# AechPro/Prism

Hardware: NVIDIA B200
Metric: PER sampled transitions/s (4 new steps ingested -> sample -> 3-step gather -> DQN update -> priority write-back, per learner iteration) (higher is better)
Workload: dtype f32

## Files before the change

### include/prism_b200.h

```cpp
#ifndef PRISM_B200_H
#define PRISM_B200_H

#include <stdint.h>

#ifdef __cplusplus
extern "C" {
#endif

#define PB_ABI_VERSION 2

enum {
    PB_OK = 0,
    PB_E_ARG = -1,
    PB_E_CAPACITY = -2,
    PB_E_UNSUPPORTED = -3,
    PB_E_POOL = -4
};

enum {
    PB_ST_EMPTY = 1,
    PB_ST_PSUM_NONPOS = 2,
    PB_ST_PMIN_NONPOS = 4
};

// ... 171 lines not shown
                         const unsigned long long *epoch, long long stride, float *partial_scratch,
                         long long *step_count, int *n_partials_out_h, void *stream);
int pb_pack_grads(int n_tensors, const long long *table, float scale, float *flat,
                  float *partial_scratch, long long *step_count, int *n_partials_out_h,
                  void *stream);
int pb_grad_sumsq(long long n, const float *grad, float *partial_scratch, long long *step_count,
                  int *n_partials_out_h, void *stream);
int pb_adam_clip_apply(long long n, float *param, const float *grad, float *exp_avg,
                       float *exp_avg_sq, const long long *step_count, float lr, float beta1,
                       float beta2, float adam_eps, float max_grad_norm,
                       const float *partial_scratch, int n_partials, float *norm_out,
                       void *stream);
long long pb_adam_fused_max_n(void);
int pb_adam_fused_step(int n_tensors, const long long *table, float scale, long long n, float *param, float *grad,
                       float *exp_avg, float *exp_avg_sq, long long *step_count, float lr, float beta1, float beta2,
                       float adam_eps, float max_grad_norm, float *partial_scratch, float *norm_out, void *stream);
int pb_adam_clip_step(long long n, float *param, const float *grad, float *exp_avg, float *exp_avg_sq,
                      long long *step_count, float lr, float beta1, float beta2, float adam_eps,
                      float max_grad_norm, float *norm_out, float *partial_scratch, void *stream);

int pb_conv3x3_relu_fwd(int B, int H, int W, int C, int OC, const float *x, const float *w,
                        const float *bias, float *out, void *stream);
int pb_conv3x3_relu_bwd_groups(int B);
int pb_conv3x3_relu_bwd(int B, int H, int W, int C, int OC, const float *x, const float *out,
                        const float *dout, float *partial_scratch, float *dw, float *db,
                        void *stream);

int pb_linear_fwd(int K, int M, int N, int J, const float *X, long long x_head_stride, const float *W,
                  const float *b, int act, float *Y, void *stream);
int pb_linear_bwd_input(int K, int M, int N, int J, const float *dY, const float *Ymask, const float *W,
                        int sum_heads, float *dX, void *stream);
int pb_linear_bwd_weight(int K, int M, int N, int J, const float *dY, const float *Ymask, const float *X,
                         long long x_head_stride, float *dW, float *db, void *stream);
int pb_gemm_trace(int enable, unsigned long long *out, int n_out);

int pb_tc_gemm_supported(int M, int N, int K, long long lda, long long ldb, long long ldc);
int pb_tc_gemm(int batch, int kbatches, int M, int N, int K,
               const float *A, int a_major, long long lda, long long a_bs,
               const float *B, int b_major, long long ldb, long long b_bs,
               const float *bias, long long bias_bs, int act,
               const float *mul, int mul_rows, long long ld_mul,
               float *C, long long ldc, long long c_bs,
               float *workspace, long long workspace_floats, int split_mode, void *stream);
int pb_linear_fwd_tc_supported(int M, int N, int J);
int pb_linear_fwd_tc(int K, int M, int N, int J, const float *X, long long x_head_stride, const float *W,
                     const float *b, int act, float *Y, void *stream);

int pb_iqn_phi_bwd(int n, int B, int F, const float *dh, const float *phi, const float *x, float *dpre, float *dx,
                   float *dbias_partial, void *stream);

#define PB_PEER_MAX 8
typedef struct pb_peer_group {
    int world, rank;
    float *grad[PB_PEER_MAX];
    float *reduced[PB_PEER_MAX];
    unsigned long long *flags[PB_PEER_MAX];
    double *norm_parts[PB_PEER_MAX];
    unsigned char *state[PB_PEER_MAX];
    unsigned long long *epoch;
    unsigned int *status;
    unsigned long long timeout_ns;
    long long grad_stride;
} pb_peer_group;
int pb_peer_alloc(long long bytes, void **ptr);
int pb_peer_free(void *ptr);
int pb_optimizer_preload(void);
// ... 75 lines not shown
```

### prism_b200/_lib.py

```python
import ctypes as C
import os

from . import build as _build

_LIB = None


class PbError(RuntimeError):
    pass


class pb_per_state(C.Structure):
    _fields_ = [
        ("len", C.c_longlong), ("seq", C.c_longlong), ("max_priority", C.c_float), ("p_sum", C.c_float),
        ("p_min", C.c_float), ("status", C.c_int), ("batch_max", C.c_float), ("owned_lo", C.c_int),
        ("owned_n", C.c_int), ("pad", C.c_int * 5),
    ]


class pb_tree(C.Structure):
    _fields_ = [
        ("sum", C.c_void_p), ("min", C.c_void_p), ("owner", C.c_void_p), ("counters", C.c_void_p),
        ("state", C.c_void_p),
        ("capacity", C.c_longlong), ("size", C.c_longlong), ("alpha", C.c_float), ("eps_f32", C.c_float),
# ... 102 lines not shown
    "pb_peer_pull_sum": [_PEER, _LL, _P, _P, C.POINTER(C.c_int), _P],
    "pb_peer_adam": [_PEER, _LL, _P, _P, _P, _P, _F, _F, _F, _F, _F, _P, _P, _P],
    "pb_peer_allreduce_adam_max_n": [],
    "pb_peer_two_phase_min": [_I],
    "pb_peer_allreduce_adam": [_PEER, _LL, _P, _P, _P, _P, _F, _F, _F, _F, _F, _P, _P, _P],
    "pb_peer_state_put": [_PEER, _P, _P],
    "pb_peer_trace": [_I, _P, _I],
    "pb_tree_sample_global_peer": [_TREE, _PEER, _LL, _P, _F, _P, _P, _P, _P],
    "pb_layer_norm_supported": [_LL, _I],
    "pb_layer_norm_bwd_blocks": [_LL, _I],
    "pb_layer_norm_fwd": [_LL, _I, _F, _P, _P, _P, _P, _P, _P, _P],
    "pb_layer_norm_bwd": [_LL, _I, _P, _P, _P, _P, _P, _P, _P, _P, _P, _P],
    "pb_layer_norm_grouped_fwd": [_I, _LL, _LL, _I, _F, _P, _P, _P, _P, _P, _P, _P],
    "pb_layer_norm_grouped_bwd_blocks": [_I, _LL, _I],
    "pb_layer_norm_grouped_bwd": [_I, _LL, _LL, _I, _P, _P, _P, _P, _P, _P, _P, _P, _P, _P],
    "pb_narrow_linear_supported": [_LL, _I, _I],
    "pb_narrow_linear_bwd_blocks": [_LL],
    "pb_narrow_linear_fwd": [_I, _LL, _I, _I, _P, _LL, _P, _P, _P, _P],
    "pb_narrow_linear_bwd": [_I, _LL, _I, _I, _P, _LL, _P, _P, _P, _P, _P, _P, _P],
    "pb_narrow_linear_bwd_reduce": [_I, _LL, _I, _I, _P, _P, _P, _P],
    "pb_sum_heads": [_I, _LL, _P, _P, _P],
    "pb_iqn_draw_cos_basis": [_LL, _I, _P, _P, _P, _P],
    "pb_relu_bwd_bias_strips": [_LL],
    "pb_relu_bwd_bias": [_I, _LL, _I, _P, _P, _P, _P, _P, _P],
    "pb_theil_chunks": [_LL],
    "pb_theil_fwd": [_I, _I, _I, _P, _P, _P, _P, _P],
    "pb_theil_bwd": [_I, _I, _I, _P, _P, _P, _P, _P],
    "pb_iqn_phi_bwd": [_I, _I, _I, _P, _P, _P, _P, _P, _P, _P],
    "pb_tc_gemm_supported": [_I, _I, _I, _LL, _LL, _LL],
    "pb_tc_gemm": [_I, _I, _I, _I, _I, _P, _I, _LL, _LL, _P, _I, _LL, _LL, _P, _LL, _I, _P, _I, _LL, _P, _LL, _LL, _P, _LL, _I, _P],
    "pb_linear_fwd_tc_supported": [_I, _I, _I],
    "pb_linear_fwd_tc": [_I, _I, _I, _I, _P, _LL, _P, _P, _I, _P, _P],
    "pb_linear_bwd_input": [_I, _I, _I, _I, _P, _P, _P, _I, _P, _P],
    "pb_linear_bwd_weight": [_I, _I, _I, _I, _P, _P, _P, _LL, _P, _P, _P],
    "pb_stamp_time": [_P, _P],
    "pb_store_stage_block": [_LL, _LL, _I, _LL, _LL, _LL, _P, _P, _P, _P, _I, _P, _P, _P, _P, _P, _P, _P, _P],
    "pb_wire_unpack_numbers": [_P, _LL, _P, _LL, _P],
    "pb_wire_array_header": [_LL, _P, _P],
    "pb_wire_pack_numbers": [_P, _I, _LL, _P, _LL, _P],
    "pb_wire_index_timesteps": [_P, _LL, _LL, _P, _P],
}
_RESTYPES = {"pb_error_string": C.c_char_p, "pb_launch_count": C.c_longlong, "pb_peer_slice": C.c_longlong,
             "pb_peer_allreduce_adam_max_n": C.c_longlong, "pb_adam_fused_max_n": C.c_longlong}

PB_E_POOL = -4
ABI_VERSION = 2


def lib_path():
    return _build.LIB_PATH


def load():
    global _LIB
    if _LIB is not None:
        return _LIB
    path = _build.build()
    if not os.path.exists(path):
        raise PbError("libprism_b200.so missing at %s and could not be built" % path)
    lib = C.CDLL(path)
    for name, argtypes in SIGNATURES.items():
        fn = getattr(lib, name)
        fn.argtypes = argtypes
        fn.restype = _RESTYPES.get(name, C.c_int)
    if lib.pb_abi_version() != ABI_VERSION:
        raise PbError("libprism_b200.so ABI version mismatch")
    _LIB = lib
    return lib


def check(rc, what=""):
    if rc != 0:
        msg = load().pb_error_string(rc).decode()
        raise PbError("%s failed: %s (code %d)" % (what or "libprism_b200 call", msg, rc))


def ptr(t):
# ... 16 lines not shown
```

### prism_b200/agents/ops.py

```python
import collections

import torch

from .. import _lib

ROUTES = collections.Counter()


def route_counts(reset=False):
    out = dict(ROUTES)
    if reset:
        ROUTES.clear()
    return out


def fallthrough_count():
    return sum(v for k, v in ROUTES.items() if k.startswith("fallthrough"))


def _c(t, dtype=torch.float32):
    if t.dtype != dtype:
        t = t.to(dtype)
    return t if t.is_contiguous() else t.contiguous()

# ... 141 lines not shown


def loss_combine(dist_loss, q_loss, per_weights):
    return _LossCombine.apply(dist_loss, q_loss, per_weights)


PARALLEL_BACKWARD = __import__('os').environ.get('PB_PARALLEL_BACKWARD', '1') != '0'
TRACE_MARK = None


def trace_mark(name):
    if TRACE_MARK is not None:
        TRACE_MARK(name)
_SIDE_STREAMS = {}


SERIAL_GRAPH = __import__('os').environ.get('PB_SERIAL_GRAPH', '0') == '1'


def fork_stream(device, key="bwd"):
    device = torch.device(device)
    if SERIAL_GRAPH:
        return torch.cuda.current_stream(device)
    s = _SIDE_STREAMS.get((device, key))
    if s is None:
        s = _SIDE_STREAMS[(device, key)] = torch.cuda.Stream(device=device)
    return s


def _side_stream(device):
    return fork_stream(device, "bwd")


_JOINS = {"mode": 0, "streams": [], "ptrs": []}


def defer_joins(mode):
    _JOINS["mode"], _JOINS["streams"], _JOINS["ptrs"] = int(mode), [], []


def finish_deferred(device):
    cur = torch.cuda.current_stream(device)
    seen = set()
    for s in _JOINS["streams"]:
        if s.cuda_stream not in seen and s.cuda_stream != cur.cuda_stream:
            seen.add(s.cuda_stream)
            cur.wait_stream(s)
    ptrs = _JOINS["ptrs"]
    defer_joins(0)
    return ptrs


def _join_or_defer(side, device, *grads):
    mode = _JOINS["mode"]
    if mode:
        _JOINS["ptrs"].extend(g.data_ptr() for g in grads if g is not None)
    if mode == 2:
        _JOINS["streams"].append(side)
    else:
        torch.cuda.current_stream(device).wait_stream(side)


class _Linear(torch.autograd.Function):

    @staticmethod
    def forward(ctx, x, w, b, act):
        _lib.require_cuda(x, "x")
        K, N, J = w.shape
        shared = x.dim() == 2
        M = x.shape[-2]
        xc, wc, bc = _c(x), _c(w), (None if b is None else _c(b))
        y = torch.empty(K, M, N, dtype=torch.float32, device=x.device)
        _lib.check(_lib.load().pb_linear_fwd(K, M, N, J, xc.data_ptr(), 0 if shared else M * J, wc.data_ptr(),
                                             _lib.ptr(bc), int(act), y.data_ptr(), _stream(x)), "pb_linear_fwd")
        ctx.act, ctx.shared, ctx.dims, ctx.has_bias = int(act), shared, (K, M, N, J), b is not None
        ctx.save_for_backward(xc, wc, y if act else None)
        return y

    @staticmethod
    def backward(ctx, dy):
        xc, wc, y = ctx.saved_tensors
        K, M, N, J = ctx.dims
        dy = _c(dy)
        lib, stream = _lib.load(), _stream(dy)
        mask = _lib.ptr(y) if ctx.act else None
        dx = dw = db = None
        want_dx = ctx.needs_input_grad[0]
        want_dw = ctx.needs_input_grad[1] or (ctx.has_bias and ctx.needs_input_grad[2])
        if want_dx:
            dx = torch.empty((M, J) if ctx.shared else (K, M, J), dtype=torch.float32, device=dy.device)
        if want_dw:
            dw = torch.empty(K, N, J, dtype=torch.float32, device=dy.device)
            db = torch.empty(K, N, dtype=torch.float32, device=dy.device) if ctx.has_bias else None
        side = _side_stream(dy.device) if (want_dx and want_dw and PARALLEL_BACKWARD) else None
        if want_dw:
            if side is not None:
                cur = torch.cuda.current_stream(dy.device)
                side.wait_stream(cur)
                with torch.cuda.stream(side):
                    _lib.check(lib.pb_linear_bwd_weight(K, M, N, J, dy.data_ptr(), mask, xc.data_ptr(),
                                                        0 if ctx.shared else M * J, dw.data_ptr(), _lib.ptr(db),
                                                        side.cuda_stream), "pb_linear_bwd_weight")
            else:
                _lib.check(lib.pb_linear_bwd_weight(K, M, N, J, dy.data_ptr(), mask, xc.data_ptr(),
                                                    0 if ctx.shared else M * J, dw.data_ptr(), _lib.ptr(db), stream),
                           "pb_linear_bwd_weight")
        if want_dx:
            _lib.check(lib.pb_linear_bwd_input(K, M, N, J, dy.data_ptr(), mask, wc.data_ptr(), int(ctx.shared),
                                               dx.data_ptr(), stream), "pb_linear_bwd_input")
        if side is not None:
            _join_or_defer(side, dy.device, dw, db)
        if TRACE_MARK is not None:
            TRACE_MARK("bwd:linear K%d M%d N%d J%d" % (K, M, N, J))
        return dx, dw, db, None


FUSED_LINEAR_MAX_ROWS = 512
NARROW_OUT, NARROW_MAX_ROWS = 32, 4096


_TC_WORKSPACE = {}
TC_WORKSPACE_FLOATS = 15 * 1024 * 1024
TC_SPLIT_MODE = 0


def _tc_workspace(device, stream):
    key = (device, stream)
    ws = _TC_WORKSPACE.get(key)
    if ws is None:
        ws = _TC_WORKSPACE[key] = torch.empty(TC_WORKSPACE_FLOATS, dtype=torch.float32, device=device)
    return ws


def tc_gemm(out, a, a_major, lda, a_bs, b, b_major, ldb, b_bs, batch, M, N, K, bias=None, bias_bs=0, act=0,
            kbatches=1, ldc=None, c_bs=None, mul=None):
    _lib.require_cuda(out, "out")
    stream = _stream(out)
    ws = _tc_workspace(out.device, stream)
    _lib.check(_lib.load().pb_tc_gemm(int(batch), int(kbatches), int(M), int(N), int(K),
                                      a.data_ptr(), int(a_major), int(lda), int(a_bs),
# ... 23 lines not shown
    @staticmethod
    def backward(ctx, dy):
        xc, wc, y = ctx.saved_tensors
        K, M, N, J = ctx.dims
        dy = _c(dy)
        lib = _lib.load()
        want_db = ctx.has_bias and ctx.needs_input_grad[2]
        dz, db = dy, None
        if ctx.act or want_db:
            strips = lib.pb_relu_bwd_bias_strips(M)
            partials = torch.empty(K * strips * N, dtype=torch.float32, device=dy.device)
            dz = torch.empty_like(dy) if ctx.act else dy
            db = torch.empty(K, N, dtype=torch.float32, device=dy.device) if want_db else None
            _lib.check(lib.pb_relu_bwd_bias(K, M, N, dy.data_ptr(), _lib.ptr(y) if ctx.act else None,
                                            dz.data_ptr() if ctx.act else None, _lib.ptr(db), partials.data_ptr(),
                                            _stream(dy)), "pb_relu_bwd_bias")
        dx = dw = None
        if ctx.needs_input_grad[0]:
            if ctx.shared:
                dx = torch.empty(M, J, dtype=torch.float32, device=dz.device)
                tc_gemm(dx, dz, 0, N, M * N, wc, 1, J, N * J, 1, M, J, N, kbatches=K)
            else:
                dx = torch.empty(K, M, J, dtype=torch.float32, device=dz.device)
                tc_gemm(dx, dz, 0, N, M * N, wc, 1, J, N * J, K, M, J, N)
        if ctx.needs_input_grad[1]:
            dw = torch.empty(K, N, J, dtype=torch.float32, device=dz.device)
            tc_gemm(dw, dz, 1, N, M * N, xc, 1, J, 0 if ctx.shared else M * J, K, N, J, M)
        return dx, dw, db, None


class _NarrowLinear(torch.autograd.Function):

    @staticmethod
    def forward(ctx, x, w, b):
        K, N, J = w.shape
        shared = x.dim() == 2
        M = x.shape[-2]
        xc, wc, bc = _c(x), _c(w), (None if b is None else _c(b))
        y = torch.empty(K, M, N, dtype=torch.float32, device=x.device)
        _lib.check(_lib.load().pb_narrow_linear_fwd(K, M, N, J, xc.data_ptr(), 0 if shared else M * J, wc.data_ptr(),
                                                    _lib.ptr(bc), y.data_ptr(), _stream(x)), "pb_narrow_linear_fwd")
        ctx.save_for_backward(xc, wc)
        ctx.has_bias, ctx.shared = b is not None, shared
        return y

    @staticmethod
    def backward(ctx, dy):
        xc, wc = ctx.saved_tensors
        K, N, J = wc.shape
        M = xc.shape[-2]
        dy = _c(dy)
        lib = _lib.load()
        want_dx, want_dw = ctx.needs_input_grad[0], ctx.needs_input_grad[1]
        want_db = ctx.has_bias and ctx.needs_input_grad[2]
        dx = torch.empty(K, M, J, dtype=torch.float32, device=dy.device) if want_dx else None
        dw = torch.empty_like(wc) if want_dw else None
        db = torch.empty(K, N, dtype=torch.float32, device=dy.device) if want_db else None
        partials = None
        if want_dw or want_db:
            partials = torch.empty(K * lib.pb_narrow_linear_bwd_blocks(M) * (N * J + N), dtype=torch.float32, device=dy.device)
        split = partials is not None and want_dx and _JOINS["mode"] and PARALLEL_BACKWARD and not SERIAL_GRAPH
        _lib.check(lib.pb_narrow_linear_bwd(K, M, N, J, xc.data_ptr(), 0 if ctx.shared else M * J, wc.data_ptr(), dy.data_ptr(),
                                            _lib.ptr(dx), None if split else _lib.ptr(dw), None if split else _lib.ptr(db),
                                            _lib.ptr(partials), _stream(dy)), "pb_narrow_linear_bwd")
        if split:
            side = _side_stream(dy.device)
            side.wait_stream(torch.cuda.current_stream(dy.device))
            with torch.cuda.stream(side):
                _lib.check(lib.pb_narrow_linear_bwd_reduce(K, M, N, J, partials.data_ptr(), _lib.ptr(dw), _lib.ptr(db),
                                                           side.cuda_stream), "pb_narrow_linear_bwd_reduce")
            _join_or_defer(side, dy.device, dw, db)
        if want_dx and ctx.shared:
            dx = sum_leading(dx)
        return dx, dw, db


NARROW_MIN_ROWS = 32


def _narrow_eligible(x, weight):
    N, J = weight.shape[-2], weight.shape[-1]
    return (x.is_cuda and x.dtype == torch.float32 and x.shape[-2] >= NARROW_MIN_ROWS
            and _lib.load().pb_narrow_linear_supported(x.shape[-2], N, J) == 1)


TENSOR_CORE_LINEAR = True
TC_MIN_ROWS = 256
TC_MIN_FLOPS = float(__import__('os').environ.get('PB_TC_MIN_FLOPS', 2.0e8))


def _tc_eligible(x, M, Kh, N, J):
    return (TENSOR_CORE_LINEAR and x.is_cuda and (J % 4) == 0 and (N % 4) == 0 and M >= TC_MIN_ROWS
            and 2.0 * M * Kh * N * J >= TC_MIN_FLOPS)


class _PhiTimesX(torch.autograd.Function):

    @staticmethod
    def forward(ctx, basis, w, b, x):
        M, J = basis.shape
        F_ = w.shape[0]
        B = x.shape[0]
        basis_c, wc, bc, xc = _c(basis), _c(w), _c(b), _c(x)
        h = torch.empty(M, F_, dtype=torch.float32, device=x.device)
        tc_gemm(h, basis_c, 0, J, 0, wc, 0, J, 0, 1, M, F_, J, bias=bc, bias_bs=0, act=1, mul=xc)
        if any(ctx.needs_input_grad[1:]):
            phi = torch.empty(M, F_, dtype=torch.float32, device=x.device)
# ... 12 lines not shown
        dx = torch.empty_like(xc) if ctx.needs_input_grad[3] else None
        dbp = torch.empty_like(xc)
        _lib.check(_lib.load().pb_iqn_phi_bwd(n, B, F_, dh.data_ptr(), phi.data_ptr(), xc.data_ptr(), dpre.data_ptr(),
                                              _lib.ptr(dx), dbp.data_ptr(), _stream(dh)), "pb_iqn_phi_bwd")
        dw = None
        if ctx.needs_input_grad[1]:
            dw = torch.empty(F_, J, dtype=torch.float32, device=dh.device)
            tc_gemm(dw, dpre, 1, F_, 0, basis_c, 1, J, 0, 1, F_, J, M)
        db = sum_leading(dbp) if ctx.needs_input_grad[2] else None
        return None, dw, db, dx


def phi_times_x(phi_seq, basis, x, n):
    import torch.nn as nn
    lin = phi_seq[0]
    M, J = basis.shape
    F_ = lin.weight.shape[0]
    if (len(phi_seq) == 2 and isinstance(lin, nn.Linear) and isinstance(phi_seq[1], nn.ReLU) and lin.bias is not None
            and x.dim() == 2 and x.shape[1] == F_ and (F_ % 4) == 0 and _tc_eligible(x, M, 1, F_, J)):
        ROUTES["phi_x:tc_gemm"] += 1
        return _PhiTimesX.apply(basis, lin.weight, lin.bias, x)
    ROUTES["fallthrough:phi_x_mul"] += 1
    phi = run_sequential(phi_seq, basis)
    return (phi.view(n, x.shape[0], -1) * x.unsqueeze(0)).view(n * x.shape[0], -1)


def linear_heads(x, w, b, relu=False):
    M, (Kh, N, J) = x.shape[-2], w.shape
    if _tc_eligible(x, M, Kh, N, J):
        ROUTES["linear:tc_gemm"] += 1
        return _LinearTC.apply(x, w, b, 1 if relu else 0)
    if not relu and N <= NARROW_OUT and _narrow_eligible(x, w):
        ROUTES["linear:narrow"] += 1
        return _NarrowLinear.apply(x, w, b)
    if x.shape[-2] > FUSED_LINEAR_MAX_ROWS:
        ROUTES["fallthrough:baddbmm"] += 1
        xe = x.unsqueeze(0).expand(w.shape[0], -1, -1) if x.dim() == 2 else x
        y = torch.baddbmm(b.unsqueeze(1), xe, w.transpose(1, 2)) if b is not None else torch.bmm(xe, w.transpose(1, 2))
        return torch.relu(y) if relu else y
    ROUTES["linear:ffma"] += 1
    return _Linear.apply(x, w, b, 1 if relu else 0)


def linear(x, weight, bias, relu=False):
    if not relu and x.dim() == 2 and weight.shape[0] <= NARROW_OUT and _narrow_eligible(x, weight):
        ROUTES["linear:narrow"] += 1
        return _NarrowLinear.apply(x, weight.unsqueeze(0), None if bias is None else bias.unsqueeze(0)).squeeze(0)
    narrow = weight.shape[0] <= NARROW_OUT and x.shape[0] <= NARROW_MAX_ROWS
    if x.shape[0] > FUSED_LINEAR_MAX_ROWS and not narrow:
        if _tc_eligible(x, x.shape[0], 1, *weight.shape):
            ROUTES["linear:tc_gemm"] += 1
            b = None if bias is None else bias.unsqueeze(0)
            return _LinearTC.apply(x, weight.unsqueeze(0), b, 1 if relu else 0).squeeze(0)
        ROUTES["fallthrough:F.linear"] += 1
        y = torch.nn.functional.linear(x, weight, bias)
        return torch.relu(y) if relu else y
    ROUTES["linear:ffma"] += 1
    b = None if bias is None else bias.unsqueeze(0)
    return _Linear.apply(x, weight.unsqueeze(0), b, 1 if relu else 0).squeeze(0)


class _LayerNorm(torch.autograd.Function):

    @staticmethod
    def forward(ctx, x, weight, bias, eps, groups, heads=False):
        xc = _c(x)
        F_ = xc.shape[-1]
# ... 250 lines not shown
```

### prism_b200/csrc/linear.cu

```cuda
#include "common.cuh"
#include <cooperative_groups.h>
#include <stdlib.h>

namespace cg = cooperative_groups;

namespace {

using namespace pb;

constexpr int TM = 64, TN = 64, TK = 32, PAD = 8;
constexpr int NS = 4;


__device__ unsigned long long g_gemm_trace[8];
__device__ int g_gemm_trace_on;
__device__ __forceinline__ void gemm_mark(int on, int slot)
{
    if (on && threadIdx.x == 0) {
        unsigned long long v;
        asm volatile("mov.u64 %0, %%globaltimer;" : "=l"(v));
        if (slot == 0) atomicMin(&g_gemm_trace[0], v); else atomicMax(&g_gemm_trace[slot], v);
    }
}

struct GemmArgs {
    const float *A, *B, *bias, *mask;
    float *C, *colsum;
    long long a_bs, b_bs, c_bs, bias_bs, colsum_bs;
    long long a_ss, b_ss;
    int lda, ldb, ldc;
    int M, N, K;
    int n_seg, splits, act, m_tiles;
};

template <bool KMAJOR>
__device__ __forceinline__ void load_tile(float (&r)[4], const float *__restrict__ P, const float *__restrict__ mask,
                                          int ld, int row0, int k0, int rows, int kmax, int t, int half)
{
    int row, k;
    if (KMAJOR) { row = row0 + (t >> 2); k = k0 + half * 16 + ((t & 3) << 2); }
    else        { k = k0 + half * 16 + (t >> 4); row = row0 + ((t & 15) << 2); }
    const bool vec_ok = (ld & 3) == 0 && ((reinterpret_cast<uintptr_t>(P) & 15) == 0);
    if (KMAJOR) {
        const long long off = (long long)row * ld + k;
        if (vec_ok && row < rows && k + 3 < kmax && (k & 3) == 0) {
            float4 v = *reinterpret_cast<const float4 *>(P + off);
            r[0] = v.x; r[1] = v.y; r[2] = v.z; r[3] = v.w;
            if (mask) {
                float4 m = *reinterpret_cast<const float4 *>(mask + off);
                r[0] = m.x > 0.f ? r[0] : 0.f; r[1] = m.y > 0.f ? r[1] : 0.f;
                r[2] = m.z > 0.f ? r[2] : 0.f; r[3] = m.w > 0.f ? r[3] : 0.f;
            }
        } else {
#pragma unroll
            for (int q = 0; q < 4; ++q) {
                float v = 0.f;
                if (row < rows && k + q < kmax) {
                    v = P[off + q];
                    if (mask && !(mask[off + q] > 0.f)) v = 0.f;
                }
                r[q] = v;
            }
        }
    } else {
        const long long off = (long long)k * ld + row;
// ... 296 lines not shown
{
    const uint32_t d = (uint32_t)__cvta_generic_to_shared(dst);
    const int n = valid ? 16 : 0;
    asm volatile("cp.async.cg.shared.global [%0], [%1], 16, %2;" ::"r"(d), "l"(src), "r"(n) : "memory");
}
__device__ __forceinline__ void cp_async_commit() { asm volatile("cp.async.commit_group;" ::: "memory"); }
template <int N>
__device__ __forceinline__ void cp_async_wait() { asm volatile("cp.async.wait_group %0;" ::"n"(N) : "memory"); }

template <bool KMAJOR>
__device__ __forceinline__ void tile_async(float *dst, const float *__restrict__ P, int ld, int row0, int k0, int rows,
                                           int kmax, int t)
{
#pragma unroll
    for (int h = 0; h < 2; ++h) {
        const int f = t + h * 256;
        if (KMAJOR) {
            const int row = f >> 3, kq = (f & 7) << 2;
            const bool ok = row0 + row < rows && k0 + kq < kmax;
            cp_async16(dst + row * RS + kq, ok ? P + (long long)(row0 + row) * ld + k0 + kq : P, ok);
        } else {
            const int k = f >> 4, rq = (f & 15) << 2;
            const bool ok = k0 + k < kmax && row0 + rq < rows;
            cp_async16(dst + k * (TM + PAD) + rq, ok ? P + (long long)(k0 + k) * ld + row0 + rq : P, ok);
        }
    }
}
template <bool KMAJOR>
__device__ __forceinline__ float tile_at(const float *tile, int row, int k)
{
    return KMAJOR ? tile[row * RS + k] : tile[k * (TM + PAD) + row];
}

template <bool A_KMAJOR, bool B_KMAJOR, bool ROWSUM, int STAGES>
__global__ void __launch_bounds__(256, STAGES == 2 ? 4 : 3) gemm_async_kernel(GemmArgs g)
{
    pdl_wait();
    pdl_trigger();
    const int tr_on = __ldg(&g_gemm_trace_on);
    gemm_mark(tr_on, 0);
    extern __shared__ __align__(16) float tiles[];
    __shared__ float Rs[TM];
    const bool masked = g.mask != nullptr;
    const int stage_words = (masked ? 3 : 2) * TILE_WORDS;
    float (*Cs)[TN + PAD] = reinterpret_cast<float (*)[TN + PAD]>(tiles);

    const int t = threadIdx.x;
    const int batch = blockIdx.y / g.m_tiles, mt = blockIdx.y % g.m_tiles;
    const int i0 = mt * TM, j0 = blockIdx.x * TN;
    const int split = blockIdx.z;
    const float *A = g.A + batch * g.a_bs, *B = g.B + batch * g.b_bs;
    const float *mask = masked ? g.mask + batch * g.a_bs : nullptr;
    const int chunks_per_seg = (g.K + TK - 1) / TK;
    const int total = g.n_seg * chunks_per_seg;
    const int per = (total + g.splits - 1) / g.splits;
    const int it0 = split * per, it1 = min(total, it0 + per);

    auto issue = [&](int it, int st) {
        if (it < it1) {
            const int seg = it / chunks_per_seg, k0 = (it % chunks_per_seg) * TK;
            float *base = tiles + st * stage_words;
            tile_async<A_KMAJOR>(base, A + seg * g.a_ss, g.lda, i0, k0, g.M, g.K, t);
            tile_async<B_KMAJOR>(base + TILE_WORDS, B + seg * g.b_ss, g.ldb, j0, k0, g.N, g.K, t);
            if (masked) tile_async<A_KMAJOR>(base + 2 * TILE_WORDS, mask + seg * g.a_ss, g.lda, i0, k0, g.M, g.K, t);
        }
        cp_async_commit();
    };
#pragma unroll
    for (int s = 0; s < STAGES; ++s) issue(it0 + s, s);

    const int lane = t & 31, gq = lane >> 2, tq = lane & 3;
    const int wm = ((t >> 5) & 3) * 16, wn = (t >> 7) * 32;
    float cf[4][4] = {};
    float acc[4][4] = {};
    float rs[4] = {};
    float rsum = 0.f;
    const bool want_rowsum = ROWSUM && g.colsum != nullptr && blockIdx.x == 0;
    const bool live = i0 + wm < g.M;

    for (int it = it0, st = 0; it < it1; ++it) {
        cp_async_wait<STAGES - 1>();
        __syncthreads();
        if (it == it0) gemm_mark(tr_on, 1);
        const float *sa = tiles + st * stage_words, *sb = sa + TILE_WORDS, *sm = sb + TILE_WORDS;
        if (live) {
#pragma unroll
            for (int k0 = 0; k0 < TK; k0 += 8) {
                float av[4] = {tile_at<A_KMAJOR>(sa, wm + gq, k0 + tq), tile_at<A_KMAJOR>(sa, wm + gq + 8, k0 + tq),
                               tile_at<A_KMAJOR>(sa, wm + gq, k0 + tq + 4), tile_at<A_KMAJOR>(sa, wm + gq + 8, k0 + tq + 4)};
                if (masked) {
                    av[0] = tile_at<A_KMAJOR>(sm, wm + gq, k0 + tq) > 0.f ? av[0] : 0.f;
                    av[1] = tile_at<A_KMAJOR>(sm, wm + gq + 8, k0 + tq) > 0.f ? av[1] : 0.f;
                    av[2] = tile_at<A_KMAJOR>(sm, wm + gq, k0 + tq + 4) > 0.f ? av[2] : 0.f;
                    av[3] = tile_at<A_KMAJOR>(sm, wm + gq + 8, k0 + tq + 4) > 0.f ? av[3] : 0.f;
                }
// ... 17 lines not shown
                const float a = tile_at<A_KMAJOR>(sa, t, k);
                rsum += (!masked || tile_at<A_KMAJOR>(sm, t, k) > 0.f) ? a : 0.f;
            }
        }
        if (it + STAGES < it1) {
            __syncthreads();
            issue(it + STAGES, st);
        } else {
            cp_async_commit();
        }
        st = st + 1 == STAGES ? 0 : st + 1;
    }
    cp_async_wait<0>();
    __syncthreads();
    gemm_mark(tr_on, 2);
    finish_tile<ROWSUM, true>(g, Cs, Rs, cf, rsum, acc, rs, batch, i0, j0, want_rowsum, tr_on);
}

int pick_splits(long long tiles, int total_chunks)
{
    static int forced = -1;
    if (forced < 0) { const char *e = getenv("PB_GEMM_SPLITS"); forced = e ? atoi(e) : 0; }
    if (forced == 1 || forced == 2 || forced == 4 || forced == 8 || forced == 16) return total_chunks >= forced ? forced : 1;
    static int max_split = -1;
    if (max_split < 0) { const char *e = getenv("PB_GEMM_MAX_SPLIT"); max_split = e ? atoi(e) : 8; }
    const int sms = pb_sm_count();
    int s = 1;
    while (s < max_split && tiles * (s * 2) <= 2LL * sms && total_chunks / (s * 2) >= 2) s *= 2;
    return s;
}

template <bool AK, bool BK, bool ROWSUM, bool FLIGHT, bool TC>
int launch_gemm_v(GemmArgs g, int batch, int n_tiles, void *stream);
template <bool AK, bool BK, bool ROWSUM, int STAGES>
int launch_gemm_async(GemmArgs g, int batch, int n_tiles, void *stream);

bool async_eligible(const GemmArgs &g, bool ak, bool bk)
{
    const uintptr_t p = reinterpret_cast<uintptr_t>(g.A) | reinterpret_cast<uintptr_t>(g.B) | reinterpret_cast<uintptr_t>(g.mask);
    if (p & 15) return false;
    if ((g.lda | g.ldb) & 3) return false;
    if ((g.a_bs | g.b_bs | g.a_ss | g.b_ss) & 3) return false;
    if (((ak ? g.K : g.M) & 3) || ((bk ? g.K : g.N) & 3)) return false;
    return true;
}

template <bool AK, bool BK, bool ROWSUM>
int launch_gemm(GemmArgs g, int batch, void *stream)
{
    g.m_tiles = (g.M + TM - 1) / TM;
    const int n_tiles = (g.N + TN - 1) / TN;
    const int total_chunks = g.n_seg * ((g.K + TK - 1) / TK);
    g.splits = pick_splits((long long)g.m_tiles * n_tiles * batch, total_chunks);
    const int per = (total_chunks + g.splits - 1) / g.splits;
    static int flight_ok = -1;
    if (flight_ok < 0) { const char *e = getenv("PB_GEMM_FLIGHT"); flight_ok = (e && e[0] == '1') ? 1 : 0; }
    static int tc_ok = -1;
    if (tc_ok < 0) { const char *e = getenv("PB_GEMM_MMA"); tc_ok = (e && e[0] == '0') ? 0 : 1; }
    const bool flight = flight_ok && per >= 3 && per <= NS;
    static int async_ok = -1;
    if (async_ok < 0) { const char *e = getenv("PB_GEMM_ASYNC"); async_ok = (e && e[0] == '0') ? 0 : 1; }
    if (tc_ok && async_ok && async_eligible(g, AK, BK)) {
        if (per <= 2) return launch_gemm_async<AK, BK, ROWSUM, 2>(g, batch, n_tiles, stream);
        return launch_gemm_async<AK, BK, ROWSUM, 4>(g, batch, n_tiles, stream);
    }
    if (tc_ok) {
        if (flight) return launch_gemm_v<AK, BK, ROWSUM, true, true>(g, batch, n_tiles, stream);
        return launch_gemm_v<AK, BK, ROWSUM, false, true>(g, batch, n_tiles, stream);
    }
    if (flight) return launch_gemm_v<AK, BK, ROWSUM, true, false>(g, batch, n_tiles, stream);
    return launch_gemm_v<AK, BK, ROWSUM, false, false>(g, batch, n_tiles, stream);
}

template <bool AK, bool BK, bool ROWSUM, bool FLIGHT, bool TC>
int launch_gemm_v(GemmArgs g, int batch, int n_tiles, void *stream)
{
    constexpr int SMEM = (FLIGHT ? NS : 2) * 2 * TK * (TM + PAD) * 4;
    if (g.splits > 8) {
        static PbPerDeviceOnce allowed;
        if (!allowed.done()) {
            cudaError_t ea = cudaFuncSetAttribute(gemm_kernel<AK, BK, ROWSUM, FLIGHT, TC>, cudaFuncAttributeNonPortableClusterSizeAllowed, 1);
            if (ea != cudaSuccess) return (int)ea;
            allowed.mark();
        }
    }
    {
        static PbPerDeviceOnce smem_set;
        if (!smem_set.done()) {
            cudaError_t es = cudaFuncSetAttribute(gemm_kernel<AK, BK, ROWSUM, FLIGHT, TC>, cudaFuncAttributeMaxDynamicSharedMemorySize, SMEM);
            if (es != cudaSuccess) return (int)es;
            smem_set.mark();
        }
    }
    cudaLaunchConfig_t cfg = {};
    cfg.gridDim = dim3((unsigned)n_tiles, (unsigned)(g.m_tiles * batch), (unsigned)g.splits);
    cfg.blockDim = dim3(256);
    cfg.dynamicSmemBytes = SMEM;
    cfg.stream = (cudaStream_t)stream;
    cudaLaunchAttribute attr[2];
    attr[0].id = cudaLaunchAttributeClusterDimension;
    attr[0].val.clusterDim.x = 1; attr[0].val.clusterDim.y = 1; attr[0].val.clusterDim.z = (unsigned)g.splits;
    attr[1].id = cudaLaunchAttributeProgrammaticStreamSerialization;
    attr[1].val.programmaticStreamSerializationAllowed = 1;
    cfg.attrs = attr;
    cfg.numAttrs = pb_pdl_chain_enabled() ? 2 : 1;
    cudaError_t e = cudaLaunchKernelEx(&cfg, gemm_kernel<AK, BK, ROWSUM, FLIGHT, TC>, g);
    g_pb_launches.fetch_add(1, std::memory_order_relaxed);
    if (e != cudaSuccess) return (int)e;
    e = cudaGetLastError();
    return e == cudaSuccess ? PB_OK : (int)e;
}

template <bool AK, bool BK, bool ROWSUM, int STAGES>
int launch_gemm_async(GemmArgs g, int batch, int n_tiles, void *stream)
{
    const int smem = STAGES * (g.mask ? 3 : 2) * TILE_WORDS * 4;
    {
        static PbPerDeviceOnce attrs_set;
        if (!attrs_set.done()) {
            cudaError_t e = cudaFuncSetAttribute(gemm_async_kernel<AK, BK, ROWSUM, STAGES>,
                                                 cudaFuncAttributeMaxDynamicSharedMemorySize, STAGES * 3 * TILE_WORDS * 4);
            if (e != cudaSuccess) return (int)e;
            e = cudaFuncSetAttribute(gemm_async_kernel<AK, BK, ROWSUM, STAGES>, cudaFuncAttributeNonPortableClusterSizeAllowed, 1);
            if (e != cudaSuccess) return (int)e;
            attrs_set.mark();
        }
    }
    cudaLaunchConfig_t cfg = {};
    cfg.gridDim = dim3((unsigned)n_tiles, (unsigned)(g.m_tiles * batch), (unsigned)g.splits);
    cfg.blockDim = dim3(256);
    cfg.dynamicSmemBytes = (size_t)smem;
    cfg.stream = (cudaStream_t)stream;
    cudaLaunchAttribute attr[2];
    attr[0].id = cudaLaunchAttributeClusterDimension;
    attr[0].val.clusterDim.x = 1; attr[0].val.clusterDim.y = 1; attr[0].val.clusterDim.z = (unsigned)g.splits;
    attr[1].id = cudaLaunchAttributeProgrammaticStreamSerialization;
    attr[1].val.programmaticStreamSerializationAllowed = 1;
    cfg.attrs = attr;
    cfg.numAttrs = pb_pdl_chain_enabled() ? 2 : 1;
    cudaError_t e = cudaLaunchKernelEx(&cfg, gemm_async_kernel<AK, BK, ROWSUM, STAGES>, g);
    g_pb_launches.fetch_add(1, std::memory_order_relaxed);
    if (e != cudaSuccess) return (int)e;
    e = cudaGetLastError();
    return e == cudaSuccess ? PB_OK : (int)e;
}

}

extern "C" {

int pb_linear_fwd(int K, int M, int N, int J, const float *X, long long x_head_stride, const float *W,
                  const float *b, int act, float *Y, void *stream)
{
    if (K <= 0 || M <= 0 || N <= 0 || J <= 0 || !X || !W || !Y || (act != 0 && act != 1)) return PB_E_ARG;
    GemmArgs g = {};
    g.A = X; g.a_bs = x_head_stride; g.lda = J;
    g.B = W; g.b_bs = (long long)N * J; g.ldb = J;
    g.C = Y; g.c_bs = (long long)M * N; g.ldc = N;
    g.bias = b; g.bias_bs = N; g.act = act;
    g.M = M; g.N = N; g.K = J; g.n_seg = 1;
    return launch_gemm<true, true, false>(g, K, stream);
}

int pb_linear_bwd_input(int K, int M, int N, int J, const float *dY, const float *Ymask, const float *W,
                        int sum_heads, float *dX, void *stream)
{
    if (K <= 0 || M <= 0 || N <= 0 || J <= 0 || !dY || !W || !dX) return PB_E_ARG;
    GemmArgs g = {};
    g.A = dY; g.mask = Ymask; g.lda = N;
    g.B = W; g.ldb = J;
    g.C = dX; g.ldc = J;
    g.M = M; g.N = J; g.K = N;
    if (sum_heads) {
        g.n_seg = K; g.a_ss = (long long)M * N; g.b_ss = (long long)N * J;
        return launch_gemm<true, false, false>(g, 1, stream);
    }
    g.n_seg = 1; g.a_bs = (long long)M * N; g.b_bs = (long long)N * J; g.c_bs = (long long)M * J;
    return launch_gemm<true, false, false>(g, K, stream);
}

int pb_linear_bwd_weight(int K, int M, int N, int J, const float *dY, const float *Ymask, const float *X,
                         long long x_head_stride, float *dW, float *db, void *stream)
{
    if (K <= 0 || M <= 0 || N <= 0 || J <= 0 || !dY || !X || !dW) return PB_E_ARG;
    GemmArgs g = {};
    g.A = dY; g.mask = Ymask; g.lda = N; g.a_bs = (long long)M * N;
    g.B = X; g.ldb = J; g.b_bs = x_head_stride;
    g.C = dW; g.ldc = J; g.c_bs = (long long)N * J;
    g.colsum = db; g.colsum_bs = N;
    g.M = N; g.N = J; g.K = M; g.n_seg = 1;
    return db ? launch_gemm<false, false, true>(g, K, stream) : launch_gemm<false, false, false>(g, K, stream);
}

int pb_gemm_trace(int enable, unsigned long long *out, int n_out)
{
    unsigned long long host[8];
    cudaError_t e = cudaDeviceSynchronize();
    if (e != cudaSuccess) return (int)e;
    e = cudaMemcpyFromSymbol(host, g_gemm_trace, sizeof(host));
    if (e != cudaSuccess) return (int)e;
    if (out) for (int k = 0; k < n_out && k < 8; ++k) out[k] = host[k];
    for (int k = 0; k < 8; ++k) host[k] = 0;
    host[0] = ~0ULL;
    e = cudaMemcpyToSymbol(g_gemm_trace, host, sizeof(host));
    if (e != cudaSuccess) return (int)e;
    const int on = enable ? 1 : 0;
    e = cudaMemcpyToSymbol(g_gemm_trace_on, &on, sizeof(on));
    return e == cudaSuccess ? PB_OK : (int)e;
}

}
// ... 1 lines not shown
```

Before: 3.462 million.

## Fuse narrow head dX recompute into preceding linear's input-gradient GEMM

When a narrow output head follows a fused linear, its backward now runs on the side stream, and the producer linear's input-gradient GEMM recomputes the head's dX tile on the fly from dQ and W2 inside the async GEMM's A-tile loader. This takes the narrow-head dX kernel off the critical path of the main stream. The cost is redundant per-tile dot products over n_out (at most 32) done with synchronous loads instead of cp.async. It also adds cross-stream bookkeeping, including tensor keep-alive in deferred joins and a fallback to waiting on the side stream when the fused path is unsupported.

Measured after the change: 3.422 million, median of 6. 1.2% lower.

```diff
diff --git a/include/prism_b200.h b/include/prism_b200.h
--- a/include/prism_b200.h
+++ b/include/prism_b200.h
@@ -227,6 +227,8 @@
                         int sum_heads, float *dX, void *stream);
 int pb_linear_bwd_weight(int K, int M, int N, int J, const float *dY, const float *Ymask, const float *X,
                          long long x_head_stride, float *dW, float *db, void *stream);
+int pb_linear_bwd_input_dq(int K, int M, int N, int J, int n_out, const float *dQ, const float *W2, const float *Ymask,
+                           const float *W, int sum_heads, float *dX, void *stream);
 int pb_gemm_trace(int enable, unsigned long long *out, int n_out);
 
 int pb_tc_gemm_supported(int M, int N, int K, long long lda, long long ldb, long long ldc);
diff --git a/prism_b200/_lib.py b/prism_b200/_lib.py
--- a/prism_b200/_lib.py
+++ b/prism_b200/_lib.py
@@ -158,6 +158,7 @@
     "pb_linear_fwd_tc_supported": [_I, _I, _I],
     "pb_linear_fwd_tc": [_I, _I, _I, _I, _P, _LL, _P, _P, _I, _P, _P],
     "pb_linear_bwd_input": [_I, _I, _I, _I, _P, _P, _P, _I, _P, _P],
+    "pb_linear_bwd_input_dq": [_I, _I, _I, _I, _I, _P, _P, _P, _P, _I, _P, _P],
     "pb_linear_bwd_weight": [_I, _I, _I, _I, _P, _P, _P, _LL, _P, _P, _P],
     "pb_stamp_time": [_P, _P],
     "pb_store_stage_block": [_LL, _LL, _I, _LL, _LL, _LL, _P, _P, _P, _P, _I, _P, _P, _P, _P, _P, _P, _P, _P],
@@ -169,6 +170,7 @@
 _RESTYPES = {"pb_error_string": C.c_char_p, "pb_launch_count": C.c_longlong, "pb_peer_slice": C.c_longlong,
              "pb_peer_allreduce_adam_max_n": C.c_longlong, "pb_adam_fused_max_n": C.c_longlong}
 
+PB_E_UNSUPPORTED = -3
 PB_E_POOL = -4
 ABI_VERSION = 2
 
diff --git a/prism_b200/agents/ops.py b/prism_b200/agents/ops.py
--- a/prism_b200/agents/ops.py
+++ b/prism_b200/agents/ops.py
@@ -197,11 +197,11 @@
     return fork_stream(device, "bwd")
 
 
-_JOINS = {"mode": 0, "streams": [], "ptrs": []}
+_JOINS = {"mode": 0, "streams": [], "ptrs": [], "keep": []}
 
 
 def defer_joins(mode):
-    _JOINS["mode"], _JOINS["streams"], _JOINS["ptrs"] = int(mode), [], []
+    _JOINS["mode"], _JOINS["streams"], _JOINS["ptrs"], _JOINS["keep"] = int(mode), [], [], []
 
 
 def finish_deferred(device):
@@ -216,14 +216,18 @@
     return ptrs
 
 
-def _join_or_defer(side, device, *grads):
+def _join_or_defer(side, device, *grads, keep=()):
     mode = _JOINS["mode"]
     if mode:
         _JOINS["ptrs"].extend(g.data_ptr() for g in grads if g is not None)
     if mode == 2:
         _JOINS["streams"].append(side)
+        _JOINS["keep"].extend(keep)
     else:
         torch.cuda.current_stream(device).wait_stream(side)
+
+
+FUSE_HEAD_BWD = __import__('os').environ.get('PB_FUSE_HEAD_BWD', '1') != '0'
 
 
 class _Linear(torch.autograd.Function):
@@ -251,6 +255,10 @@
         mask = _lib.ptr(y) if ctx.act else None
         dx = dw = db = None
         want_dx = ctx.needs_input_grad[0]
+        pend, ctx.pb_dq = getattr(ctx, "pb_dq", None), None
+        if pend is not None and dy.data_ptr() != pend[2].data_ptr():
+            torch.cuda.current_stream(dy.device).wait_stream(_side_stream(dy.device))
+            pend = None
         want_dw = ctx.needs_input_grad[1] or (ctx.has_bias and ctx.needs_input_grad[2])
         if want_dx:
             dx = torch.empty((M, J) if ctx.shared else (K, M, J), dtype=torch.float32, device=dy.device)
@@ -260,8 +268,7 @@
         side = _side_stream(dy.device) if (want_dx and want_dw and PARALLEL_BACKWARD) else None
         if want_dw:
             if side is not None:
-                cur = torch.cuda.current_stream(dy.device)
-                side.wait_stream(cur)
+                side.wait_stream(torch.cuda.current_stream(dy.device))
                 with torch.cuda.stream(side):
                     _lib.check(lib.pb_linear_bwd_weight(K, M, N, J, dy.data_ptr(), mask, xc.data_ptr(),
                                                         0 if ctx.shared else M * J, dw.data_ptr(), _lib.ptr(db),
@@ -270,7 +277,17 @@
                 _lib.check(lib.pb_linear_bwd_weight(K, M, N, J, dy.data_ptr(), mask, xc.data_ptr(),
                                                     0 if ctx.shared else M * J, dw.data_ptr(), _lib.ptr(db), stream),
                            "pb_linear_bwd_weight")
-        if want_dx:
+        rc = _lib.PB_E_UNSUPPORTED
+        if want_dx and pend is not None:
+            dq, w2 = pend[0], pend[1]
+            rc = lib.pb_linear_bwd_input_dq(K, M, N, J, w2.shape[1], dq.data_ptr(), w2.data_ptr(), mask, wc.data_ptr(),
+                                            int(ctx.shared), dx.data_ptr(), stream)
+            if rc == _lib.PB_E_UNSUPPORTED:
+                torch.cuda.current_stream(dy.device).wait_stream(_side_stream(dy.device))
+            else:
+                _lib.check(rc, "pb_linear_bwd_input_dq")
+                ROUTES["linear:bwd_input_dq"] += 1
+        if want_dx and rc == _lib.PB_E_UNSUPPORTED:
             _lib.check(lib.pb_linear_bwd_input(K, M, N, J, dy.data_ptr(), mask, wc.data_ptr(), int(ctx.shared),
                                                dx.data_ptr(), stream), "pb_linear_bwd_input")
         if side is not None:
@@ -360,7 +377,7 @@
 class _NarrowLinear(torch.autograd.Function):
 
     @staticmethod
-    def forward(ctx, x, w, b):
+    def forward(ctx, x, w, b, producer=None):
         K, N, J = w.shape
         shared = x.dim() == 2
         M = x.shape[-2]
@@ -370,6 +387,7 @@
                                                     _lib.ptr(bc), y.data_ptr(), _stream(x)), "pb_narrow_linear_fwd")
         ctx.save_for_backward(xc, wc)
         ctx.has_bias, ctx.shared = b is not None, shared
+        ctx.producer = None if shared else producer
         return y
 
     @staticmethod
@@ -387,6 +405,18 @@
         partials = None
         if want_dw or want_db:
             partials = torch.empty(K * lib.pb_narrow_linear_bwd_blocks(M) * (N * J + N), dtype=torch.float32, device=dy.device)
+        prod, ctx.producer = ctx.producer, None
+        if (prod is not None and want_dx and any(prod.needs_input_grad) and FUSE_HEAD_BWD and PARALLEL_BACKWARD
+                and not SERIAL_GRAPH):
+            side = _side_stream(dy.device)
+            side.wait_stream(torch.cuda.current_stream(dy.device))
+            with torch.cuda.stream(side):
+                _lib.check(lib.pb_narrow_linear_bwd(K, M, N, J, xc.data_ptr(), M * J, wc.data_ptr(), dy.data_ptr(),
+                                                    dx.data_ptr(), _lib.ptr(dw), _lib.ptr(db), _lib.ptr(partials),
+                                                    side.cuda_stream), "pb_narrow_linear_bwd")
+            prod.pb_dq = (dy, wc, dx)
+            _join_or_defer(side, dy.device, dw, db, keep=(dx, partials))
+            return dx, dw, db, None
         split = partials is not None and want_dx and _JOINS["mode"] and PARALLEL_BACKWARD and not SERIAL_GRAPH
         _lib.check(lib.pb_narrow_linear_bwd(K, M, N, J, xc.data_ptr(), 0 if ctx.shared else M * J, wc.data_ptr(), dy.data_ptr(),
                                             _lib.ptr(dx), None if split else _lib.ptr(dw), None if split else _lib.ptr(db),
@@ -400,7 +430,7 @@
             _join_or_defer(side, dy.device, dw, db)
         if want_dx and ctx.shared:
             dx = sum_leading(dx)
-        return dx, dw, db
+        return dx, dw, db, None
 
 
 NARROW_MIN_ROWS = 32
@@ -479,7 +509,8 @@
         return _LinearTC.apply(x, w, b, 1 if relu else 0)
     if not relu and N <= NARROW_OUT and _narrow_eligible(x, w):
         ROUTES["linear:narrow"] += 1
-        return _NarrowLinear.apply(x, w, b)
+        producer = x.grad_fn if isinstance(x.grad_fn, _Linear._backward_cls) else None
+        return _NarrowLinear.apply(x, w, b, producer)
     if x.shape[-2] > FUSED_LINEAR_MAX_ROWS:
         ROUTES["fallthrough:baddbmm"] += 1
         xe = x.unsqueeze(0).expand(w.shape[0], -1, -1) if x.dim() == 2 else x
diff --git a/prism_b200/csrc/linear.cu b/prism_b200/csrc/linear.cu
--- a/prism_b200/csrc/linear.cu
+++ b/prism_b200/csrc/linear.cu
@@ -31,6 +31,8 @@
     int lda, ldb, ldc;
     int M, N, K;
     int n_seg, splits, act, m_tiles;
+    const float *dq, *w2;
+    int n_out;
 };
 
 template <bool KMAJOR>
@@ -393,7 +395,26 @@
     return KMAJOR ? tile[row * RS + k] : tile[k * (TM + PAD) + row];
 }
 
-template <bool A_KMAJOR, bool B_KMAJOR, bool ROWSUM, int STAGES>
+__device__ __forceinline__ void dq_tile(float *dst, const GemmArgs &g, int head, int row0, int k0, int t)
+{
+    const float *dq = g.dq + (size_t)head * g.M * g.n_out, *w2 = g.w2 + (size_t)head * g.n_out * g.K;
+#pragma unroll
+    for (int h = 0; h < 2; ++h) {
+        const int f = t + h * 256, row = f >> 3, kq = (f & 7) << 2;
+        float4 d = make_float4(0.f, 0.f, 0.f, 0.f);
+        if (row0 + row < g.M && k0 + kq < g.K) {
+            const float *q = dq + (size_t)(row0 + row) * g.n_out, *w = w2 + k0 + kq;
+            for (int n = 0; n < g.n_out; ++n) {
+                const float qn = __ldg(q + n);
+                const float4 wn = __ldg(reinterpret_cast<const float4 *>(w + (size_t)n * g.K));
+                d.x = fmaf(qn, wn.x, d.x); d.y = fmaf(qn, wn.y, d.y); d.z = fmaf(qn, wn.z, d.z); d.w = fmaf(qn, wn.w, d.w);
+            }
+        }
+        *reinterpret_cast<float4 *>(dst + row * RS + kq) = d;
+    }
+}
+
+template <bool A_KMAJOR, bool B_KMAJOR, bool ROWSUM, int STAGES, bool DQ = false>
 __global__ void __launch_bounds__(256, STAGES == 2 ? 4 : 3) gemm_async_kernel(GemmArgs g)
 {
     pdl_wait();
@@ -421,7 +442,8 @@
         if (it < it1) {
             const int seg = it / chunks_per_seg, k0 = (it % chunks_per_seg) * TK;
             float *base = tiles + st * stage_words;
-            tile_async<A_KMAJOR>(base, A + seg * g.a_ss, g.lda, i0, k0, g.M, g.K, t);
+            if constexpr (DQ) dq_tile(base, g, batch + seg, i0, k0, t);
+            else tile_async<A_KMAJOR>(base, A + seg * g.a_ss, g.lda, i0, k0, g.M, g.K, t);
             tile_async<B_KMAJOR>(base + TILE_WORDS, B + seg * g.b_ss, g.ldb, j0, k0, g.N, g.K, t);
             if (masked) tile_async<A_KMAJOR>(base + 2 * TILE_WORDS, mask + seg * g.a_ss, g.lda, i0, k0, g.M, g.K, t);
         }
@@ -505,7 +527,7 @@
 
 template <bool AK, bool BK, bool ROWSUM, bool FLIGHT, bool TC>
 int launch_gemm_v(GemmArgs g, int batch, int n_tiles, void *stream);
-template <bool AK, bool BK, bool ROWSUM, int STAGES>
+template <bool AK, bool BK, bool ROWSUM, int STAGES, bool DQ = false>
 int launch_gemm_async(GemmArgs g, int batch, int n_tiles, void *stream);
 
 bool async_eligible(const GemmArgs &g, bool ak, bool bk)
@@ -516,6 +538,19 @@
     if ((g.a_bs | g.b_bs | g.a_ss | g.b_ss) & 3) return false;
     if (((ak ? g.K : g.M) & 3) || ((bk ? g.K : g.N) & 3)) return false;
     return true;
+}
+
+bool tc_products_on()
+{
+    static int tc_ok = -1;
+    if (tc_ok < 0) { const char *e = getenv("PB_GEMM_MMA"); tc_ok = (e && e[0] == '0') ? 0 : 1; }
+    return tc_ok;
+}
+bool async_kernel_on()
+{
+    static int async_ok = -1;
+    if (async_ok < 0) { const char *e = getenv("PB_GEMM_ASYNC"); async_ok = (e && e[0] == '0') ? 0 : 1; }
+    return tc_products_on() && async_ok;
 }
 
 template <bool AK, bool BK, bool ROWSUM>
@@ -528,12 +563,9 @@
     const int per = (total_chunks + g.splits - 1) / g.splits;
     static int flight_ok = -1;
     if (flight_ok < 0) { const char *e = getenv("PB_GEMM_FLIGHT"); flight_ok = (e && e[0] == '1') ? 1 : 0; }
-    static int tc_ok = -1;
-    if (tc_ok < 0) { const char *e = getenv("PB_GEMM_MMA"); tc_ok = (e && e[0] == '0') ? 0 : 1; }
+    const bool tc_ok = tc_products_on();
     const bool flight = flight_ok && per >= 3 && per <= NS;
-    static int async_ok = -1;
-    if (async_ok < 0) { const char *e = getenv("PB_GEMM_ASYNC"); async_ok = (e && e[0] == '0') ? 0 : 1; }
-    if (tc_ok && async_ok && async_eligible(g, AK, BK)) {
+    if (async_kernel_on() && async_eligible(g, AK, BK)) {
         if (per <= 2) return launch_gemm_async<AK, BK, ROWSUM, 2>(g, batch, n_tiles, stream);
         return launch_gemm_async<AK, BK, ROWSUM, 4>(g, batch, n_tiles, stream);
     }
@@ -584,17 +616,17 @@
     return e == cudaSuccess ? PB_OK : (int)e;
 }
 
-template <bool AK, bool BK, bool ROWSUM, int STAGES>
+template <bool AK, bool BK, bool ROWSUM, int STAGES, bool DQ>
 int launch_gemm_async(GemmArgs g, int batch, int n_tiles, void *stream)
 {
     const int smem = STAGES * (g.mask ? 3 : 2) * TILE_WORDS * 4;
     {
         static PbPerDeviceOnce attrs_set;
         if (!attrs_set.done()) {
-            cudaError_t e = cudaFuncSetAttribute(gemm_async_kernel<AK, BK, ROWSUM, STAGES>,
+            cudaError_t e = cudaFuncSetAttribute(gemm_async_kernel<AK, BK, ROWSUM, STAGES, DQ>,
                                                  cudaFuncAttributeMaxDynamicSharedMemorySize, STAGES * 3 * TILE_WORDS * 4);
             if (e != cudaSuccess) return (int)e;
-            e = cudaFuncSetAttribute(gemm_async_kernel<AK, BK, ROWSUM, STAGES>, cudaFuncAttributeNonPortableClusterSizeAllowed, 1);
+            e = cudaFuncSetAttribute(gemm_async_kernel<AK, BK, ROWSUM, STAGES, DQ>, cudaFuncAttributeNonPortableClusterSizeAllowed, 1);
             if (e != cudaSuccess) return (int)e;
             attrs_set.mark();
         }
@@ -611,7 +643,7 @@
     attr[1].val.programmaticStreamSerializationAllowed = 1;
     cfg.attrs = attr;
     cfg.numAttrs = pb_pdl_chain_enabled() ? 2 : 1;
-    cudaError_t e = cudaLaunchKernelEx(&cfg, gemm_async_kernel<AK, BK, ROWSUM, STAGES>, g);
+    cudaError_t e = cudaLaunchKernelEx(&cfg, gemm_async_kernel<AK, BK, ROWSUM, STAGES, DQ>, g);
     g_pb_launches.fetch_add(1, std::memory_order_relaxed);
     if (e != cudaSuccess) return (int)e;
     e = cudaGetLastError();
@@ -650,6 +682,28 @@
     }
     g.n_seg = 1; g.a_bs = (long long)M * N; g.b_bs = (long long)N * J; g.c_bs = (long long)M * J;
     return launch_gemm<true, false, false>(g, K, stream);
+}
+
+int pb_linear_bwd_input_dq(int K, int M, int N, int J, int n_out, const float *dQ, const float *W2, const float *Ymask,
+                           const float *W, int sum_heads, float *dX, void *stream)
+{
+    if (K <= 0 || M <= 0 || N <= 0 || J <= 0 || n_out <= 0 || !dQ || !W2 || !W || !dX) return PB_E_ARG;
+    GemmArgs g = {};
+    g.A = dQ; g.mask = Ymask; g.lda = N;
+    g.B = W; g.ldb = J;
+    g.C = dX; g.ldc = J;
+    g.M = M; g.N = J; g.K = N;
+    g.dq = dQ; g.w2 = W2; g.n_out = n_out;
+    if (sum_heads) { g.n_seg = K; g.a_ss = (long long)M * N; g.b_ss = (long long)N * J; }
+    else { g.n_seg = 1; g.a_bs = (long long)M * N; g.b_bs = (long long)N * J; g.c_bs = (long long)M * J; }
+    if (n_out > 32 || (reinterpret_cast<uintptr_t>(W2) & 15) || !async_kernel_on() || !async_eligible(g, true, false))
+        return PB_E_UNSUPPORTED;
+    const int batch = sum_heads ? 1 : K;
+    g.m_tiles = (M + TM - 1) / TM;
+    const int n_tiles = (J + TN - 1) / TN, total_chunks = g.n_seg * ((N + TK - 1) / TK);
+    g.splits = pick_splits((long long)g.m_tiles * n_tiles * batch, total_chunks);
+    if (total_chunks <= 2 * g.splits) return launch_gemm_async<true, false, false, 2, true>(g, batch, n_tiles, stream);
+    return launch_gemm_async<true, false, false, 4, true>(g, batch, n_tiles, stream);
 }
 
 int pb_linear_bwd_weight(int K, int M, int N, int J, const float *dY, const float *Ymask, const float *X,
```
